# rasd3/TODA

Measured on AMD Instinct MI355X. Metric: LiDAR training samples/sec, higher is better.
Workload: dtype f32

## Files before the change

### include/toda.h

```cpp
#ifndef TODA_H_
#define TODA_H_

#include <stddef.h>
#include <stdint.h>

#ifdef __cplusplus
extern "C" {
#endif

#define TODA_OK 0
#define TODA_EINVAL (-1)
#define TODA_EWORKSPACE (-2)
#define TODA_ELAUNCH (-3)
#define TODA_EFAULT (-4)

#define TODA_FAULT_BN2D 1u
#define TODA_FAULT_WINO 2u
#define TODA_FAULT_FPS 4u

const char* toda_last_error(void);
int toda_abi_version(void);
int toda_device_fault(void);

size_t toda_voxelize_workspace_bytes(int n_points, int max_voxels);
// ... 232 lines not shown
                     const double* hi_xy_host, int closed, int32_t* flags, void* stream);
int toda_points_polar_cell(const float* points, int n, const int32_t* n_dev, int c, float phase,
                           const double* yaw_edges_host, int n_yaw, const double* dis_edges_host, int n_dis,
                           float dis_lo, float dis_hi, int32_t* cell, void* stream);
int toda_points_polar_select(const float* points, int n, const int32_t* n_dev, int c, double lo, double hi, int yaw_mode,
                             int dis_mode, double dis_th, const float* pitch_range_dev, int32_t* flags, void* stream);
size_t toda_points_pitch_range_workspace_bytes(void);
int toda_points_pitch_range(const float* points, int n, const int32_t* n_dev, int c, float* range_dev, void* ws,
                            size_t ws_bytes, void* stream);
int toda_points_pitch_band(const float* points, int n, const int32_t* n_dev, int c, float z_offset, float clip_lo,
                           float clip_hi, const double* edges_host, int n_bands, int32_t* band, void* stream);
size_t toda_rows_select_workspace_bytes(int n);
int toda_rows_select_append(const float* src, int n, const int32_t* n_dev, int c, const int32_t* keys,
                            int match, int invert, float* dst, int cap_rows, int32_t* cursor_dev,
                            void* ws, size_t ws_bytes, void* stream);
int toda_points_rotate_z(const float* src, int n, const int32_t* n_dev, int c, double cosv, double sinv,
                         float* dst, void* stream);
int toda_points_world_transform(const float* src, int n, const int32_t* n_dev, int c, int flip_x, int flip_y,
                                int rotate, float cosv, float sinv, int rescale, float scale, float* dst,
                                void* stream);

int toda_spconv_gather_gemm_stats_supported(int c_gather, int c_produce);
size_t toda_spconv_gather_gemm_stats_doubles(int n_out, int c_produce);
int toda_spconv_gather_gemm_stats(const float* in, int n_in, int c_gather, const float* packed_w, const int32_t* nbr,
                                  int n_out, int k_vol, int c_produce, const float* bias, float* out, double* sums,
                                  size_t sums_doubles, void* stream);
int toda_spconv_gather_gemm_stats_partials(const float* in, int n_in, int c_gather, const float* wp, const int32_t* nbr,
                                           int n_out, int k_vol, int c_produce, const float* bias , float* out,
                                           double* sums, size_t sums_doubles, int* blocks_out, void* stream);

int toda_conv3x3_supported(int batch, int cin, int cout, int H, int W);
size_t toda_conv3x3_weight_floats(int cout, int cin);
int toda_conv3x3_transform_weight(const float* w, int cout, int cin, int mode, float* u, void* stream);
size_t toda_conv3x3_workspace_bytes(void);
size_t toda_conv3x3_wgrad_workspace_bytes(int batch, int cin, int cout, int H, int W);
int toda_conv3x3_wgrad(const float* x, const float* dy, int batch, int cin, int cout, int H, int W, float* dw,
                       void* ws, size_t ws_bytes, void* stream);
int toda_conv3x3_fwd(const float* x, const float* u, const float* bias, int batch, int cin, int cout, int H,
                     int W, float* y, void* ws, size_t ws_bytes, void* stream);

int toda_conv3x3s2_supported(int batch, int cin, int cout, int H, int W);
int toda_conv3x3s2_fwd(const float* x, const float* w, int batch, int cin, int cout, int H, int W, float* y, void* stream);
int toda_conv3x3s2_dgrad(const float* dy, const float* w, int batch, int cin, int cout, int H, int W, float* dx, void* stream);
size_t toda_conv3x3s2_wgrad_workspace_bytes(int batch, int cin, int cout, int H, int W);
int toda_conv3x3s2_wgrad(const float* x, const float* dy, int batch, int cin, int cout, int H, int W, float* dw, void* ws,
                         size_t ws_bytes, void* stream);
int toda_deconv_supported(int batch, int cin, int cout, int H, int W, int s);
int toda_deconv_fwd(const float* x, const float* w, int batch, int cin, int cout, int H, int W, int s, float* y, void* stream);
int toda_deconv_dgrad(const float* dy, const float* w, int batch, int cin, int cout, int H, int W, int s, float* dx, void* stream);
size_t toda_deconv_wgrad_workspace_bytes(int batch, int cin, int cout, int H, int W, int s);
int toda_deconv_wgrad(const float* x, const float* dy, int batch, int cin, int cout, int H, int W, int s, float* dw, void* ws,
                      size_t ws_bytes, void* stream);

size_t toda_center_loss_workspace_bytes(int batch, int classes, int H, int W, int max_objs, int code_size);
int toda_center_loss_fwd(const float* hm_logits, const float* heatmap, int batch, int classes, int H, int W, int n_branch,
                         const float* const* reg_maps_host, const int32_t* reg_channels_host, const int64_t* inds,
                         const int64_t* mask, const float* target_boxes, int max_objs, int code_size,
                         const float* code_weights_host, float cls_weight, float loc_weight, float* hm_prob, float* out4,
                         void* ws, size_t ws_bytes, void* stream);
int toda_center_loss_bwd(const float* out4, const float* up_hm, const float* up_loc, int batch, int classes, int H, int W,
                         int n_branch, float* const* reg_grads_host, const int32_t* reg_channels_host, const int64_t* inds,
                         const int64_t* mask, int max_objs, int code_size, const float* code_weights_host, float cls_weight, float loc_weight,
                         float* hm_grad, const void* ws, size_t ws_bytes, void* stream);

int toda_conv3x3_narrow_supported(int batch, int cin, int cout, int H, int W);
int toda_conv3x3_narrow_fwd(int n, const float* const* x_host, const float* const* w_host, const float* const* bias_host,
// ... 37 lines not shown
```

### toda_amd/csrc/conv2d.hip

```cpp
#include <hip/hip_ext.h>
#include <stdlib.h>

#include "common.h"

#ifndef TODA_ABLATE
#define TODA_ABLATE 0
#endif

namespace toda {

typedef float f32x4 __attribute__((ext_vector_type(4)));
typedef float f32x2 __attribute__((ext_vector_type(2)));
typedef unsigned int u32x4w __attribute__((ext_vector_type(4)));

constexpr int WN_BLOCK = 256;
constexpr int WN_TILES = 32;
constexpr int WN_COUT = 32;
constexpr int WN_KC = 8;
constexpr int WN_FREQ = 36;
constexpr int WN_IMG = 256;
constexpr unsigned WN_OOB = 0xFFFFFFF0u;

struct WinoGeom {
    int B, Cin, Cout, H, W;
    int tiles_x, tiles_y, tiles_img, n_tiles;
    int n_tile_blocks, n_cout_blocks, n_chunks;
};

__device__ __constant__ double WN_G[6][3] = {
    {1.0, 0.0, 0.0},
    {-1.0 / 3, 1.0 / 3, -1.0 / 3},
    {1.0 / 3, 1.0 / 3, 1.0 / 3},
    {-16.0 / 15, -8.0 / 15, -4.0 / 15},
    {1.0 / 15, -2.0 / 15, 4.0 / 15},
// ... 1 lines not shown
};

__device__ __forceinline__ void wn_bt(float d0, float d1, float d2, float d3, float d4, float d5, float& v0, float& v1,
                                      float& v2, float& v3, float& v4, float& v5) {
    const float a = d3 - d1, b = d4 - d2;
    v0 = __builtin_fmaf(1.5f, a, __builtin_fmaf(-2.0f, d2, d0 + d4));
    v1 = __builtin_fmaf(-2.5f, d2, __builtin_fmaf(0.5f, d3, d1 + d4));
    v2 = __builtin_fmaf(2.5f, d3, __builtin_fmaf(0.5f, d2, d4 - d1));
    v3 = __builtin_fmaf(2.0f, a, b);
    v4 = __builtin_fmaf(-0.5f, a, b);
    v5 = __builtin_fmaf(1.5f, b, __builtin_fmaf(-2.0f, d3, d1 + d5));
}

__device__ __forceinline__ void wn_at(float m0, float m1, float m2, float m3, float m4, float m5, float& y0, float& y1,
                                      float& y2, float& y3) {
    const float s = m1 + m2, d = m2 - m1;
    y0 = (m0 + s) + (m3 + m4);
    y1 = __builtin_fmaf(-2.0f, m4, __builtin_fmaf(0.5f, m3, d));
    y2 = __builtin_fmaf(4.0f, m4, __builtin_fmaf(0.25f, m3, s));
    y3 = __builtin_fmaf(-8.0f, m4, __builtin_fmaf(0.125f, m3, d)) + m5;
}

__device__ __forceinline__ void wn_a(float y0, float y1, float y2, float y3, float& m0, float& m1, float& m2, float& m3,
                                     float& m4, float& m5) {
    const float e = y0 + y2, o = y1 + y3;
    m0 = y0;
    m1 = e - o;
    m2 = e + o;
    m3 = __builtin_fmaf(0.125f, y3, __builtin_fmaf(0.25f, y2, __builtin_fmaf(0.5f, y1, y0)));
    m4 = __builtin_fmaf(-8.0f, y3, __builtin_fmaf(4.0f, y2, __builtin_fmaf(-2.0f, y1, y0)));
    m5 = y3;
}

__global__ void __launch_bounds__(WN_BLOCK)
wino_weight_kernel(const float* __restrict__ w, int cout, int cin, int mode, float* __restrict__ u) {
    const unsigned per = (unsigned)6 * cout * cin;
    unsigned e = blockIdx.x * WN_BLOCK + threadIdx.x;
    if (e >= (mode == 2 ? 2 * per : per)) return;
    const int md = mode == 2 ? (e >= per ? 1 : 0) : mode;
    float* dst = u;
    if (e >= per) {
        e -= per;
        dst += (size_t)WN_FREQ * cout * cin;
    }
    const int CI = md ? cout : cin;
    const unsigned n_chunks = (unsigned)CI >> 3;
    const int s_ = (int)(e & 1), n = (int)((e >> 1) & 15), j = (int)((e >> 5) & 3), wc = (int)((e >> 7) & 1);
    unsigned t = e >> 8;
    const int fi = (int)(t % 6u);
    t /= 6u;
    const int chunk = (int)(t % n_chunks), cb = (int)(t / n_chunks);
    const int co = cb * 32 + wc * 16 + n, ci = chunk * 8 + 2 * j + s_;
    const float* const gp = w + (md ? ((size_t)ci * cin + co) : ((size_t)co * cin + ci)) * 9;
    double tb[3];
#pragma unroll
    for (int b2 = 0; b2 < 3; ++b2) {
        double acc = 0.0;
#pragma unroll
        for (int a = 0; a < 3; ++a) acc += WN_G[fi][a] * (double)(md ? gp[(2 - a) * 3 + (2 - b2)] : gp[a * 3 + b2]);
        tb[b2] = acc;
    }
    dst += ((size_t)(cb * n_chunks + chunk) * WN_FREQ + fi * 6) * WN_IMG + (e & 255u);
#pragma unroll
    for (int fj = 0; fj < 6; ++fj) dst[(size_t)fj * WN_IMG] = (float)(tb[0] * WN_G[fj][0] + tb[1] * WN_G[fj][1] + tb[2] * WN_G[fj][2]);
}

__device__ __forceinline__ __amdgpu_buffer_rsrc_t wn_rsrc(const float* base, unsigned bytes) {
    return __builtin_amdgcn_make_buffer_rsrc(const_cast<float*>(base), 0, bytes, 0x00020000);
}

__device__ __forceinline__ int wn_work_id() {
    const int nwg = gridDim.x, xcd = blockIdx.x & 7, q8 = nwg >> 3, r8 = nwg & 7;
    return (xcd < r8 ? xcd * (q8 + 1) : r8 * (q8 + 1) + (xcd - r8) * q8) + (blockIdx.x >> 3);
}

struct PatchOff {
    unsigned offc[6];
    unsigned offe[6];
    bool left, right;
    bool tail;
};

__device__ __forceinline__ PatchOff wn_patch_off(int tile, int t, int chan, int C, const WinoGeom& g) {
    PatchOff p;
    const bool exists = tile < g.n_tiles;
    const int tl = exists ? tile : 0;
    const int b = tl / g.tiles_img, rem = tl - b * g.tiles_img;
    const int ty = rem / g.tiles_x, tx = rem - ty * g.tiles_x;
    const int y0 = 4 * ty, x0 = 4 * tx;
    const int base = ((b * C + chan) * g.H + (y0 - 1)) * g.W + x0;
    const bool has_l = x0 > 0, has_r = x0 + 4 < g.W;
    p.left = has_l || t == 0;
    p.right = has_r || t == 15;
    p.tail = x0 + 3 >= g.W;
#pragma unroll
    for (int r = 0; r < 6; ++r) {
        const int yy = y0 - 1 + r;
// ... 701 lines not shown
                float* const d0 = lds + buf * IMG + img_off;
                float* const d1 = lds + (2 + buf) * IMG + img_off;
#pragma unroll
                for (int f = 0; f < WN_FREQ; ++f) {
                    d0[f * WN_IMG] = st.x.c[f % 6][f & 3];
                    d1[f * WN_IMG] = st.y.c[f & 3][f % 4];
                }
                return;
            }
            wn_x_transform_store(st.x, lds + buf * IMG + img_off);
            wn_dy_transform_store(st.y, lds + (2 + buf) * IMG + img_off);
        };
        auto barrier = [&]() { asm volatile("s_waitcnt lgkmcnt(0)\n\ts_barrier" ::: "memory"); };
        WStage s0, s1;
        fetch(s0, 0);
        fetch(s1, 1);
        produce(s0, 0);
        int q = 0;
        while (true) {
            barrier();
            if (q + 1 >= total) break;
            fetch(s0, q + 2);
            produce(s1, (q + 1) & 1);
            ++q;
            barrier();
            if (q + 1 >= total) break;
            fetch(s1, q + 2);
            produce(s0, (q + 1) & 1);
            ++q;
        }
    }
}

template <int SLAB>
__global__ void __launch_bounds__(WN_BLOCK)
wino_wgrad_reduce_kernel(const float* __restrict__ slabs, const int n_units, const int steps_per_unit, int G, float* __restrict__ red) {
    static_assert(SLAB % WN_BLOCK == 0, "a fold block must not straddle two units");
    __shared__ int seg[WS_MAX_GRID];
    __shared__ int n_seg;
    const long long e = (long long)blockIdx.x * WN_BLOCK + threadIdx.x;
    const int unit = (int)(((long long)blockIdx.x * WN_BLOCK) / SLAB);
    if (threadIdx.x == 0) {
        const long long S = (long long)n_units * steps_per_unit;
        const long long u_lo = (long long)unit * steps_per_unit, u_hi = u_lo + steps_per_unit;
        int w0 = (int)(u_lo * G / S);
        while (w0 > 0 && ws_range_lo(w0, G, S) > u_lo) --w0;
        while (w0 + 1 < G && ws_range_lo(w0 + 1, G, S) <= u_lo) ++w0;
        int n = 0;
        long long lo = ws_range_lo(w0, G, S);
        for (int w = w0; w < G && lo < u_hi; ++w) {
            const long long next = ws_range_lo(w + 1, G, S);
            if (next > u_lo && next != lo) seg[n++] = w;
            lo = next;
        }
        n_seg = n;
    }
    __syncthreads();
    if (unit >= n_units) return;
    const int off = (int)(e - (long long)unit * SLAB);
    const float* p = slabs + (size_t)unit * SLAB + off;
    const int n = n_seg;
    float acc = 0.0f;
    int i = 0;
    for (; i + 8 <= n; i += 8) {
        float v[8];
#pragma unroll
        for (int j = 0; j < 8; ++j) v[j] = p[(size_t)seg[i + j] * SLAB];
#pragma unroll
        for (int j = 0; j < 8; ++j) acc += v[j];
    }
    for (; i < n; ++i) acc += p[(size_t)seg[i] * SLAB];
    red[e] = acc;
}

__global__ void __launch_bounds__(WN_BLOCK)
wino_wgrad_finish_kernel(const float* __restrict__ red, const WgradGeom wg, float* __restrict__ dw) {
    const int e = blockIdx.x * WN_BLOCK + threadIdx.x;
    const int cin = wg.g.Cin, cout = wg.g.Cout;
    if (e >= cin * cout) return;
    const int co = e / cin, ci = e - co * cin;
    const int unit = (ci >> 5) * wg.n_co_blocks + (co >> 5);
    const float* sl = red + (size_t)unit * WG_SLAB_FLOATS + (co & 31) * 32 + (ci & 31);
    double du[WN_FREQ];
#pragma unroll
    for (int f = 0; f < WN_FREQ; ++f) du[f] = (double)sl[f * 1024];
    double t[3][6];
#pragma unroll
    for (int a = 0; a < 3; ++a)
#pragma unroll
        for (int j = 0; j < 6; ++j) {
            double acc = 0.0;
#pragma unroll
            for (int i = 0; i < 6; ++i) acc += WN_G[i][a] * du[i * 6 + j];
            t[a][j] = acc;
        }
    float* out = dw + ((size_t)co * cin + ci) * 9;
#pragma unroll
    for (int a = 0; a < 3; ++a)
#pragma unroll
        for (int b = 0; b < 3; ++b) {
            double acc = 0.0;
#pragma unroll
            for (int j = 0; j < 6; ++j) acc += t[a][j] * WN_G[j][b];
            out[a * 3 + b] = (float)acc;
        }
}


static int wino_geom(const char* who, int batch, int cin, int cout, int H, int W, WinoGeom* g) {
    TODA_CHECK_ARG(batch >= 1 && H >= 1 && W >= 2 && W % 2 == 0, "%s: needs batch >= 1, H >= 1 and an even W (got %d x %d x %d)", who, batch, H, W);
    TODA_CHECK_ARG(cin >= WN_KC && cin % WN_KC == 0, "%s: input channels must be a multiple of %d (got %d)", who, WN_KC, cin);
    TODA_CHECK_ARG(cout >= WN_COUT && cout % WN_COUT == 0, "%s: output channels must be a multiple of %d (got %d)", who, WN_COUT, cout);
    const long long in_bytes = 4LL * batch * cin * H * W, out_bytes = 4LL * batch * cout * H * W;
    TODA_CHECK_ARG(in_bytes < (1LL << 32) - 65536 && out_bytes < (1LL << 32) - 65536, "%s: tensor above 4 GiB", who);
    g->B = batch, g->Cin = cin, g->Cout = cout, g->H = H, g->W = W;
    g->tiles_x = (W + 3) / 4, g->tiles_y = (H + 3) / 4;
    g->tiles_img = g->tiles_x * g->tiles_y;
    g->n_tiles = batch * g->tiles_img;
    g->n_tile_blocks = cdiv(g->n_tiles, WN_TILES);
    g->n_cout_blocks = cout / WN_COUT;
    g->n_chunks = cin / WN_KC;
    return TODA_OK;
}

}

using namespace toda;

extern "C" size_t toda_conv3x3_weight_floats(int cout, int cin) {
    return (size_t)WN_FREQ * cout * cin;
}

extern "C" int toda_conv3x3_supported(int batch, int cin, int cout, int H, int W) {
    if (batch < 1 || H < 1 || W < 2 || (W & 1)) return 0;
    if (cin < 32 || cin % 32 || cout < 32 || cout % 32) return 0;
    if (4LL * batch * (cin > cout ? cin : cout) * H * W >= (1LL << 32) - 65536) return 0;
    return 1;
}

extern "C" int toda_conv3x3_transform_weight(const float* w, int cout, int cin, int mode, float* u, void* stream) {
    TODA_CHECK_ARG(w && u && mode >= 0 && mode <= 2, "conv3x3_transform_weight: null pointer or bad mode");
    const int CO = mode == 1 ? cin : cout, CI = mode == 1 ? cout : cin;
    TODA_CHECK_ARG(CO % WN_COUT == 0 && CI % WN_KC == 0 && CO > 0 && CI > 0 && (mode != 2 || (CI % WN_COUT == 0)),
                   "conv3x3_transform_weight: produced channels %% 32 and contracted channels %% 8 must be 0 (got %d, %d)", CO, CI);
    const long long threads = 6LL * cout * cin * (mode == 2 ? 2 : 1);
    TODA_CHECK_ARG(threads * 6 < (1LL << 31), "conv3x3_transform_weight: operand above 2^31 elements");
    hipLaunchKernelGGL(wino_weight_kernel, dim3(cdiv(threads, WN_BLOCK)), dim3(WN_BLOCK), 0, (hipStream_t)stream, w, cout, cin, mode, u);
    TODA_LAUNCH_CHECK();
    return TODA_OK;
}

extern "C" size_t toda_conv3x3_workspace_bytes(void) {
    return WS_FLAG_BYTES + (size_t)WS_MAX_GRID * WS_SLAB_FLOATS * sizeof(float);
}

extern "C" int toda_conv3x3_fwd(const float* x, const float* u, const float* bias, int batch, int cin, int cout, int H, int W,
                                float* y, void* ws, size_t ws_bytes, void* stream) {
    TODA_CHECK_ARG(x && u && y, "conv3x3_fwd: null pointer");
    WinoGeom g;
    int rc = wino_geom("conv3x3_fwd", batch, cin, cout, H, W, &g);
    if (rc) return rc;
    static const int variant = getenv("TODA_WINO_VARIANT") ? atoi(getenv("TODA_WINO_VARIANT")) : 1;
    const int n_units = g.n_tile_blocks * g.n_cout_blocks;
    if (variant == 0) {
        hipLaunchKernelGGL(wino_fwd_kernel, dim3(n_units), dim3(WN_BLOCK), 0, (hipStream_t)stream, x, u, bias, y, g);
    } else {
        TODA_CHECK_ARG(ws != nullptr, "conv3x3_fwd: workspace missing");
        if (ws_bytes < toda_conv3x3_workspace_bytes()) {
            toda::set_error("conv3x3_fwd: workspace too small (%zu < %zu bytes)", ws_bytes, toda_conv3x3_workspace_bytes());
            return TODA_EWORKSPACE;
        }
        static int n_cu = 0;
        if (!n_cu) {
            int dev = 0;
            hipDeviceProp_t prop;
            TODA_HIP(hipGetDevice(&dev));
            TODA_HIP(hipGetDeviceProperties(&prop, dev));
            n_cu = prop.multiProcessorCount > 0 ? prop.multiProcessorCount : 256;
            if (n_cu > WS_MAX_GRID) n_cu = WS_MAX_GRID;
        }
        static const int env_gang = getenv("TODA_WINO_GANG") ? atoi(getenv("TODA_WINO_GANG")) : 1;
        static const int gang_kb = getenv("TODA_WINO_GANG_KB") ? atoi(getenv("TODA_WINO_GANG_KB")) : 2560;
// ... 37 lines not shown


extern "C" size_t toda_conv3x3_wgrad_workspace_bytes(int batch, int cin, int cout, int H, int W) {
    (void)batch, (void)H, (void)W;
    const size_t units = (size_t)(cin / 32) * (cout / 32);
    return (WS_MAX_GRID + 2 * units) * WG_SLAB_FLOATS * sizeof(float);
}

extern "C" int toda_conv3x3_wgrad(const float* x, const float* dy, int batch, int cin, int cout, int H, int W, float* dw, void* ws,
                                  size_t ws_bytes, void* stream) {
    TODA_CHECK_ARG(x && dy && dw, "conv3x3_wgrad: null pointer");
    WgradGeom wg;
    int rc = wgrad_geom("conv3x3_wgrad", batch, cin, cout, H, W, &wg);
    if (rc) return rc;
    const size_t need = toda_conv3x3_wgrad_workspace_bytes(batch, cin, cout, H, W);
    if (!ws || ws_bytes < need) {
        toda::set_error("conv3x3_wgrad: workspace too small (%zu < %zu bytes)", ws_bytes, need);
        return TODA_EWORKSPACE;
    }
    static int n_cu = 0;
    if (!n_cu) {
        int dev = 0;
        hipDeviceProp_t prop;
        TODA_HIP(hipGetDevice(&dev));
        TODA_HIP(hipGetDeviceProperties(&prop, dev));
        n_cu = prop.multiProcessorCount > 0 ? prop.multiProcessorCount : 256;
        if (n_cu > WS_MAX_GRID) n_cu = WS_MAX_GRID;
    }
    const long long steps = (long long)wg.n_units * wg.steps_per_unit;
    const int grid = steps < n_cu ? (int)steps : n_cu;
    static const int ablate = (TODA_ABLATE && getenv("TODA_WINO_WG_ABLATE")) ? atoi(getenv("TODA_WINO_WG_ABLATE")) : 0;
    hipLaunchKernelGGL(wino_wgrad_kernel, dim3(grid), dim3(WS_BLOCK), 0, (hipStream_t)stream, x, dy, wg, (float*)ws, ablate);
    TODA_LAUNCH_CHECK();
    float* red = (float*)ws + (size_t)(WS_MAX_GRID + wg.n_units) * WG_SLAB_FLOATS;
    hipLaunchKernelGGL(wino_wgrad_reduce_kernel<WG_SLAB_FLOATS>, dim3(cdiv((long long)wg.n_units * WG_SLAB_FLOATS, WN_BLOCK)), dim3(WN_BLOCK), 0,
                       (hipStream_t)stream, (const float*)ws, wg.n_units, wg.steps_per_unit, grid, red);
    TODA_LAUNCH_CHECK();
    hipLaunchKernelGGL(wino_wgrad_finish_kernel, dim3(cdiv((long long)cin * cout, WN_BLOCK)), dim3(WN_BLOCK), 0, (hipStream_t)stream,
                       (const float*)red, wg, dw);
    TODA_LAUNCH_CHECK();
    return TODA_OK;
}
```

### toda_amd/lib.py

```python
import ctypes as C
import os

import torch

_HERE = os.path.dirname(os.path.abspath(__file__))
LIB_PATH = os.environ.get("TODA_HIP_LIB") or os.path.join(_HERE, "libtoda_hip.so")

_vp, _i, _sz, _dbl = C.c_void_p, C.c_int, C.c_size_t, C.c_double

SIGNATURES = {
    "toda_last_error": (C.c_char_p, []),
    "toda_abi_version": (_i, []),
    "toda_device_fault": (_i, []),
    "toda_voxelize_workspace_bytes": (_sz, [_i, _i]),
    "toda_voxelize_hard": (_i, [_vp, _i, _i, _vp, _vp, _vp, _i, _i, _vp, _vp, _vp, _vp, _vp, _sz, _vp]),
    "toda_mean_vfe_fwd": (_i, [_vp, _vp, _i, _i, _i, _vp, _vp]),
    "toda_mean_vfe_bwd": (_i, [_vp, _vp, _i, _i, _i, _vp, _vp]),
    "toda_dynvox_workspace_bytes": (_sz, [_i, _i, _vp, _i]),
    "toda_dynvox_count": (_i, [_vp, _i, _i, _i, _vp, _vp, _vp, _i, _vp, _vp, _sz, _vp]),
    "toda_dynvox_index": (_i, [_vp, _i, _i, _i, _vp, _vp, _vp, _i, _i, _i, _vp, _vp, _vp, _vp, _vp, _vp, _vp, _vp, _sz, _vp]),
    "toda_dynvox_seg_sum": (_i, [_vp, _i, _i, _i, _vp, _vp, _vp, _i, _i, _vp, _vp]),
    "toda_dynvox_pillar_decorate": (_i, [_vp, _i, _vp, _vp, _vp, _vp, _i, _vp, _vp, _i, _i, _vp, _i, _vp]),
    "toda_dynvox_seg_max_fwd": (_i, [_vp, _i, _vp, _vp, _i, _vp, _vp, _vp]),
    "toda_dynvox_seg_max_bwd": (_i, [_vp, _vp, _i, _i, _i, _vp, _vp]),
# ... 71 lines not shown
    "toda_voxel_pool_table": (_i, [_vp, _vp, _i, _i, _i, _vp, _vp, _vp, _sz, _vp]),
    "toda_voxel_pool_bwd_feat": (_i, [_vp, _vp, _i, _i, _i, _vp, _vp, _i, _vp, _vp]),
    "toda_voxel_pool_bwd_pos_doubles": (_sz, [_i]),
    "toda_voxel_pool_bwd_pos": (_i, [_vp, _vp, _vp, _vp, _i, _i, _i, _vp, _i, _vp, _vp, _vp, _vp]),
    "toda_fps_resident_blocks": (_i, []),
    "toda_fps_workspace_bytes": (_sz, [_i, _i]),
    "toda_fps": (_i, [_vp, _vp, _i, _i, _i, _vp, _vp, _vp, _sz, _vp]),
    "toda_ball_query_stack": (_i, [_vp, _i, _vp, _vp, _vp, _i, _i, _i, _vp, _vp, _vp, _vp, _vp]),
    "toda_sa_gather_fwd": (_i, [_vp, _i, _i, _vp, _vp, _vp, _i, _i, _vp, _vp, _vp, _vp]),
    "toda_sa_gather_bwd_feat": (_i, [_vp, _i, _i, _i, _vp, _vp, _i, _vp, _vp]),
    "toda_sa_gather_bwd_pos_doubles": (_sz, [_i]),
    "toda_sa_gather_bwd_pos": (_i, [_vp, _vp, _vp, _i, _i, _i, _vp, _i, _vp, _vp, _vp, _vp]),
    "toda_sa_max_fwd": (_i, [_vp, _i, _i, _i, _vp, _vp, _vp]),
    "toda_sa_max_bwd": (_i, [_vp, _vp, _i, _i, _i, _vp, _vp]),
    "toda_bev_interp_fwd": (_i, [_vp, _i, _i, _i, _i, _vp, _vp, _i, _vp, _vp, _vp, _vp]),
    "toda_bev_interp_bwd": (_i, [_vp, _i, _i, _vp, _vp, _vp, _i, _i, _i, _vp, _vp]),
    "toda_clip_adam_chunk": (_i, []),
    "toda_clip_adam_step": (_i, [_vp, _vp, _vp, _vp, _vp, _vp, _vp, _i, _vp, _vp, C.c_float, C.c_float, C.c_float, C.c_float, C.c_float, C.c_float, _i, _vp]),
    "toda_points_in_boxes": (_i, [_vp, _i, _vp, _i, _vp, _i, _i, _i, _vp, _vp]),
    "toda_points_sector": (_i, [_vp, _i, _vp, _i, _dbl, _dbl, _vp, _vp]),
    "toda_points_rect": (_i, [_vp, _i, _vp, _i, _vp, _vp, _i, _vp, _vp]),
    "toda_points_polar_cell": (_i, [_vp, _i, _vp, _i, C.c_float, _vp, _i, _vp, _i, C.c_float, C.c_float, _vp, _vp]),
    "toda_points_polar_select": (_i, [_vp, _i, _vp, _i, _dbl, _dbl, _i, _i, _dbl, _vp, _vp, _vp]),
    "toda_points_pitch_range_workspace_bytes": (_sz, []),
    "toda_points_pitch_range": (_i, [_vp, _i, _vp, _i, _vp, _vp, _sz, _vp]),
    "toda_points_pitch_band": (_i, [_vp, _i, _vp, _i, C.c_float, C.c_float, C.c_float, _vp, _i, _vp, _vp]),
    "toda_rows_select_workspace_bytes": (_sz, [_i]),
    "toda_rows_select_append": (_i, [_vp, _i, _vp, _i, _vp, _i, _i, _vp, _i, _vp, _vp, _sz, _vp]),
    "toda_points_rotate_z": (_i, [_vp, _i, _vp, _i, _dbl, _dbl, _vp, _vp]),
    "toda_points_world_transform": (_i, [_vp, _i, _vp, _i, _i, _i, _i, C.c_float, C.c_float, _i, C.c_float, _vp, _vp]),
    "toda_conv3x3_supported": (_i, [_i, _i, _i, _i, _i]),
    "toda_conv3x3_weight_floats": (_sz, [_i, _i]),
    "toda_conv3x3_transform_weight": (_i, [_vp, _i, _i, _i, _vp, _vp]),
    "toda_conv3x3_workspace_bytes": (_sz, []),
    "toda_conv3x3_wgrad_workspace_bytes": (_sz, [_i, _i, _i, _i, _i]),
    "toda_conv3x3_wgrad": (_i, [_vp, _vp, _i, _i, _i, _i, _i, _vp, _vp, _sz, _vp]),
    "toda_conv3x3_fwd": (_i, [_vp, _vp, _vp, _i, _i, _i, _i, _i, _vp, _vp, _sz, _vp]),
    "toda_conv3x3_narrow_supported": (_i, [_i, _i, _i, _i, _i]),
    "toda_conv3x3_narrow_fwd": (_i, [_i, _vp, _vp, _vp, _vp, _i, _i, _i, _i, C.c_longlong, _vp, _vp]),
    "toda_conv3x3_narrow_dgrad": (_i, [_i, _vp, _vp, _vp, _i, _i, _i, _i, C.c_longlong, _vp, _vp]),
    "toda_conv3x3_narrow_wgrad_workspace_bytes": (_sz, [_i, _i, _i, _i]),
    "toda_conv3x3_narrow_wgrad": (_i, [_i, _vp, _vp, _vp, _i, _i, _i, _i, C.c_longlong, _vp, _vp, _sz, _vp]),
    "toda_center_loss_workspace_bytes": (_sz, [_i, _i, _i, _i, _i, _i]),
    "toda_center_loss_fwd": (_i, [_vp, _vp, _i, _i, _i, _i, _i, _vp, _vp, _vp, _vp, _vp, _i, _i, _vp, C.c_float, C.c_float, _vp, _vp, _vp, _sz, _vp]),
    "toda_center_loss_bwd": (_i, [_vp, _vp, _vp, _i, _i, _i, _i, _i, _vp, _vp, _vp, _vp, _i, _i, _vp, C.c_float, C.c_float, _vp, _vp, _sz, _vp]),
    "toda_timing_begin": (_i, [_i]),
    "toda_timing_end": (_i, [_vp, _i, _vp]),
    "toda_center_assign": (_i, [_vp, _i, _i, _i, _i, _i, _i, _vp, _vp, _i, _i, _dbl, _i, _vp, _vp, _vp, _vp, _vp]),
    "toda_anchor_assign_workspace_bytes": (_sz, [_i, _i]),
    "toda_anchor_assign": (_i, [_vp, _vp, _vp, _vp, _vp, _i, _i, _vp, _i, _i, _i, _vp, _i, _i, _i, _i, _vp, _vp, _vp, _vp, _sz, _vp]),
    "toda_eval_overlaps": (_i, [_vp, _vp, _vp, _vp, _vp, _vp, _vp, _i, C.c_longlong, _i, _i, _vp, _vp]),
    "toda_eval_match_workspace_bytes": (_sz, [_i, _i, _i]),
    "toda_eval_match_scores": (_i, [_vp, _vp, _vp, _vp, _vp, _vp, _vp, _i, _i, _dbl, _vp, _vp, _vp, _sz, _vp]),
    "toda_eval_match": (_i, [_vp, _vp, _vp, _vp, _vp, _vp, _vp, _vp, _vp, _vp, _vp, _vp, _i, _i, _vp, _i, _dbl, _i, _i, _vp, _vp, _sz, _vp]),
}

_lib = None


def load():
    global _lib
    if _lib is not None:
        return _lib
    if not os.path.exists(LIB_PATH):
        raise RuntimeError(
            f"{LIB_PATH} not found: build it with `python -c 'import __graft_entry__ as g; g.build()'` "
# ... 38 lines not shown


def stream():
    if _raw_stream is not None and _raw_device is not None:
        return _raw_stream(_raw_device())
    return torch.cuda.current_stream().cuda_stream


def host_ptrs(tensors):
    return (C.c_void_p * len(tensors))(*[ptr(t) for t in tensors])


def host_addrs(addrs):
    return (C.c_void_p * len(addrs))(*[int(a) for a in addrs])


def host_i32(vals):
    arr = (C.c_int32 * len(vals))(*[int(v) for v in vals])
    return arr


def host_f32(vals):
    arr = (C.c_float * len(vals))(*[float(v) for v in vals])
    return arr


def host_f64(vals):
    arr = (C.c_double * len(vals))(*[float(v) for v in vals])
    return arr


def hptr(arr):
    return C.cast(arr, C.c_void_p)
```

### toda_amd/ops.py

```python
import numpy as np
import torch

from . import arena as _arena
from . import lib as L


def _triple(v):
    if isinstance(v, (list, tuple)):
        assert len(v) == 3
        return [int(x) for x in v]
    return [int(v)] * 3


def grid_size_xyz(pc_range, voxel_size):
    r = np.asarray(pc_range, dtype=np.float64)
    return np.round((r[3:6] - r[0:3]) / np.asarray(voxel_size, dtype=np.float64)).astype(np.int64)


import os as _os
import time as _time

_COUNT_PINNED = {}
_LAST_WAIT_S = 0.0

# ... 1090 lines not shown
BN2D_CAT = _os.environ.get("TODA_BN2D_CAT", "1") == "1"


def bn2d_supported(x, bn):
    if not (FUSED_BN2D and type(bn) is torch.nn.BatchNorm2d and bn.training and bn.affine and bn.track_running_stats and bn.momentum is not None):
        return False
    if not (x.is_cuda and x.dtype == torch.float32 and x.dim() == 4 and x.is_contiguous()):
        return False
    return bool(L.load().toda_bn2d_supported(x.shape[0], x.shape[1], x.shape[2] * x.shape[3]))


def bn2d(x, bn, relu):
    bump_bn_counter(bn)
    return _BN2d.apply(x, bn.weight, bn.bias, bn.running_mean, bn.running_var, bn.momentum, bn.eps, relu)


def bn2d_cat(pairs, relu=True):
    flat = []
    for x, bn in pairs:
        bump_bn_counter(bn)
        flat += [x, bn.weight, bn.bias, bn.running_mean, bn.running_var, bn.momentum, bn.eps]
    return _BN2dCat.apply(relu, len(pairs), *flat)


def bn_relu_tail(seq):
    mods = list(seq)
    if len(mods) >= 2 and type(mods[-1]) is torch.nn.ReLU and type(mods[-2]) is torch.nn.BatchNorm2d:
        return mods[:-2], mods[-2]
    return None


def run_dense_sequential(seq, x):
    mods = list(seq)
    i = 0
    while i < len(mods):
        m = mods[i]
        if isinstance(m, torch.nn.Sequential):
            x = run_dense_sequential(m, x)
        elif (type(m) is torch.nn.ZeroPad2d and tuple(m.padding) == (1, 1, 1, 1) and i + 1 < len(mods) and type(mods[i + 1]) is torch.nn.Conv2d
              and mods[i + 1].padding == (0, 0) and conv3x3_supported(x, mods[i + 1])):
            x = conv3x3(x, mods[i + 1].weight, mods[i + 1].bias)
            i += 2
            continue
        elif (type(m) is torch.nn.ZeroPad2d and tuple(m.padding) == (1, 1, 1, 1) and i + 1 < len(mods) and conv3x3s2_supported(x, mods[i + 1])):
            x = conv3x3s2(x, mods[i + 1].weight, mods[i + 1].bias)
            i += 2
            continue
        elif deconv_supported(x, m):
            x = deconv(x, m.weight, m.stride[0], m.bias)
        elif type(m) is torch.nn.Conv2d and m.padding == (1, 1) and conv3x3_supported(x, m):
            x = conv3x3(x, m.weight, m.bias)
        elif type(m) is torch.nn.BatchNorm2d and bn2d_supported(x, m):
            relu = i + 1 < len(mods) and type(mods[i + 1]) is torch.nn.ReLU
            x = bn2d(x, m, relu)
            i += 2 if relu else 1
            continue
        elif type(m) is torch.nn.BatchNorm2d and x.is_cuda and m.track_running_stats and m.momentum is not None:
            bump_bn_counter(m)
            x = torch.nn.functional.batch_norm(x, m.running_mean, m.running_var, m.weight, m.bias, m.training, m.momentum, m.eps)
        else:
            x = m(x)
        i += 1
    return x


DENSE_CONV = _os.environ.get("TODA_DENSE_CONV", "winograd")
_WINO_CACHE = {}


def conv3x3_supported(x, conv):
    if DENSE_CONV != "winograd" or type(conv) is not torch.nn.Conv2d or not x.is_cuda or x.dtype != torch.float32 or x.dim() != 4:
        return False
    if conv.kernel_size != (3, 3) or conv.stride != (1, 1) or conv.dilation != (1, 1) or conv.groups != 1:
        return False
    if conv.padding_mode != "zeros" or conv.in_channels != x.shape[1]:
        return False
    b, c, h, w = x.shape
    return bool(L.load().toda_conv3x3_supported(b, conv.in_channels, conv.out_channels, h, w))


def conv3x3_transform_weight(weight, mode):
    lib = L.load()
    cout, cin = weight.shape[0], weight.shape[1]
    n = lib.toda_conv3x3_weight_floats(cout, cin)
    u = torch.empty((2, n) if mode == 2 else (n,), dtype=torch.float32, device=weight.device)
    L.check(lib.toda_conv3x3_transform_weight(L.ptr(weight.contiguous()), cout, cin, int(mode), L.ptr(u), L.stream()),
            "toda_conv3x3_transform_weight")
    return u


def _conv3x3_workspace(device):
    key = (device.index, L.stream())
    ws = _WINO_CACHE.get(key)
    if ws is None:
        ws = _WINO_CACHE[key] = torch.zeros((L.load().toda_conv3x3_workspace_bytes(),), dtype=torch.uint8, device=device)
    return ws


def conv3x3_run(x, u, bias, cout):
    lib = L.load()
    b, cin, h, w = x.shape
    y = torch.empty((b, cout, h, w), dtype=torch.float32, device=x.device)
    ws = _conv3x3_workspace(x.device)
    L.check(lib.toda_conv3x3_fwd(L.ptr(x), L.ptr(u), L.ptr(bias), b, cin, cout, h, w, L.ptr(y), L.ptr(ws), ws.numel(), L.stream()),
            "toda_conv3x3_fwd")
    return y


class _Conv3x3(torch.autograd.Function):

    @staticmethod
    def forward(ctx, x, weight, bias):
        x = x.contiguous()
        need_dx = ctx.needs_input_grad[0]
        u = conv3x3_transform_weight(weight, 2 if need_dx else 0)
        y = conv3x3_run(x, u[0] if need_dx else u, bias, weight.shape[0])
        ctx.save_for_backward(x, weight, u[1] if need_dx else None)
        ctx.has_bias = bias is not None
        return y

    @staticmethod
    def backward(ctx, gy):
        x, weight, u_dgrad = ctx.saved_tensors
        gy = gy.contiguous()
        gx = gw = gb = None
        if ctx.needs_input_grad[0]:
            gx = conv3x3_run(gy, u_dgrad if u_dgrad is not None else conv3x3_transform_weight(weight, 1), None, weight.shape[1])
        if ctx.needs_input_grad[1]:
            gw = conv3x3_wgrad(x, gy, weight.shape)
        if ctx.has_bias and ctx.needs_input_grad[2]:
            gb = gy.sum((0, 2, 3))
        return gx, gw, gb


def conv3x3_wgrad(x, gy, wshape):
    lib = L.load()
    b, cin, h, w = x.shape
    cout = gy.shape[1]
    dw = torch.empty(tuple(wshape), dtype=torch.float32, device=x.device)
    ws_bytes = lib.toda_conv3x3_wgrad_workspace_bytes(b, cin, cout, h, w)
    ws = torch.empty((max(ws_bytes, 16),), dtype=torch.uint8, device=x.device)
    L.check(lib.toda_conv3x3_wgrad(L.ptr(x), L.ptr(gy), b, cin, cout, h, w, L.ptr(dw), L.ptr(ws), ws_bytes, L.stream()),
            "toda_conv3x3_wgrad")
    return dw


def conv3x3(x, weight, bias=None):
    return _Conv3x3.apply(x, weight, bias)


class _Conv3x3S2(torch.autograd.Function):

    @staticmethod
    def forward(ctx, x, weight):
        lib = L.load()
        x, weight = x.contiguous(), weight.contiguous()
        b, cin, h, w = x.shape
        cout = weight.shape[0]
        y = torch.empty((b, cout, h // 2, w // 2), dtype=torch.float32, device=x.device)
        L.check(lib.toda_conv3x3s2_fwd(L.ptr(x), L.ptr(weight), b, cin, cout, h, w, L.ptr(y), L.stream()), "toda_conv3x3s2_fwd")
        ctx.save_for_backward(x, weight)
        return y

    @staticmethod
    def backward(ctx, gy):
        x, weight = ctx.saved_tensors
        lib = L.load()
        gy = gy.contiguous()
        b, cin, h, w = x.shape
        cout = weight.shape[0]
        gx = gw = None
        if ctx.needs_input_grad[0]:
            gx = torch.empty_like(x)
            L.check(lib.toda_conv3x3s2_dgrad(L.ptr(gy), L.ptr(weight), b, cin, cout, h, w, L.ptr(gx), L.stream()), "toda_conv3x3s2_dgrad")
        if ctx.needs_input_grad[1]:
            gw = torch.empty_like(weight)
            nb = lib.toda_conv3x3s2_wgrad_workspace_bytes(b, cin, cout, h, w)
            ws = torch.empty((max(nb, 16),), dtype=torch.uint8, device=x.device)
            L.check(lib.toda_conv3x3s2_wgrad(L.ptr(x), L.ptr(gy), b, cin, cout, h, w, L.ptr(gw), L.ptr(ws), nb, L.stream()), "toda_conv3x3s2_wgrad")
        return gx, gw

# ... 862 lines not shown
```

### toda_amd/pcdet/models/backbones_2d/base_bev_backbone.py

```python
import numpy as np
import torch
import torch.nn as nn

from toda_amd import ops


def _bn(c):
    return nn.BatchNorm2d(c, eps=1e-3, momentum=0.01)


class BaseBEVBackbone(nn.Module):
    def __init__(self, model_cfg, input_channels):
        super().__init__()
        self.model_cfg = model_cfg
        layer_nums = list(model_cfg.get("LAYER_NUMS", None) or [])
        layer_strides = list(model_cfg.get("LAYER_STRIDES", None) or [])
        num_filters = list(model_cfg.get("NUM_FILTERS", None) or [])
        assert len(layer_nums) == len(layer_strides) == len(num_filters)
        up_strides = list(model_cfg.get("UPSAMPLE_STRIDES", None) or [])
        up_filters = list(model_cfg.get("NUM_UPSAMPLE_FILTERS", None) or [])
        assert len(up_strides) == len(up_filters)

        self.blocks, self.deblocks = nn.ModuleList(), nn.ModuleList()
        c_prev = input_channels
        for lvl, (n_layers, stride, width) in enumerate(zip(layer_nums, layer_strides, num_filters)):
            seq = [nn.ZeroPad2d(1), nn.Conv2d(c_prev, width, 3, stride=stride, padding=0, bias=False), _bn(width),
                   nn.ReLU()]
            for _ in range(n_layers):
                seq += [nn.Conv2d(width, width, 3, padding=1, bias=False), _bn(width), nn.ReLU()]
            self.blocks.append(nn.Sequential(*seq))
            c_prev = width
            if up_strides:
                s = up_strides[lvl]
                if s >= 1:
                    up = nn.ConvTranspose2d(width, up_filters[lvl], s, stride=s, bias=False)
                else:
                    k = int(np.round(1 / s))
                    up = nn.Conv2d(width, up_filters[lvl], k, stride=k, bias=False)
                self.deblocks.append(nn.Sequential(up, _bn(up_filters[lvl]), nn.ReLU()))
        c_cat = sum(up_filters)
        if len(up_strides) > len(layer_nums):
            s = up_strides[-1]
            self.deblocks.append(nn.Sequential(nn.ConvTranspose2d(c_cat, c_cat, s, stride=s, bias=False), _bn(c_cat),
                                               nn.ReLU()))
        self.num_bev_features = c_cat

    def forward(self, data_dict):
        x = data_dict["spatial_features"]
        if getattr(self, "dense_channels_last", False):
            x = x.contiguous(memory_format=torch.channels_last)
        h0 = x.shape[2]
        ups, pre = [], []
        tails = [ops.bn_relu_tail(d) for d in self.deblocks[:len(self.blocks)]] if (ops.BN2D_CAT and len(self.blocks) > 1 and len(self.deblocks) >= len(self.blocks)) else []
        for lvl, block in enumerate(self.blocks):
            x = ops.run_dense_sequential(block, x)
            data_dict[f"spatial_features_{int(h0 / x.shape[2])}x"] = x
            if tails and all(t is not None for t in tails):
                pre.append((ops.run_dense_sequential(tails[lvl][0], x), tails[lvl][1]))
            else:
                ups.append(ops.run_dense_sequential(self.deblocks[lvl], x) if len(self.deblocks) > 0 else x)
        if pre:
            if all(ops.bn2d_supported(z, bn) for z, bn in pre) and len({z.shape[2:] for z, _ in pre}) == 1:
                x = ops.bn2d_cat(pre, relu=True)
            else:
                ups = [torch.relu(ops.run_dense_sequential([bn], z)) for z, bn in pre]
        if len(ups) > 1:
            x = torch.cat(ups, dim=1)
        elif len(ups) == 1:
            x = ups[0]
        if len(self.deblocks) > len(self.blocks):
            x = ops.run_dense_sequential(self.deblocks[-1], x)
        data_dict["spatial_features_2d"] = x
        return data_dict
```

Measured before the change: 146.8.

## Batch Winograd weight transforms across layers and fuse wgrad reduce with filter fold

Adds a batched weight-transform kernel that handles up to 16 conv3x3 layers in one launch, plus a Python prepack pass that caches the transformed weights per conv, keyed on weight version, pointer and a manual epoch. It also adds a wgrad fold kernel that sums the per-workgroup slabs and applies the inverse filter transform in a single kernel, replacing the separate reduce and transform launches. The intent is to cut kernel launches and host overhead in the BEV backbone. The cache is invalidated only through the weight version and pointer and an explicit epoch bump, so in-place weight writes that skip the version counter could leave stale transformed weights.

```diff
diff --git a/include/toda.h b/include/toda.h
--- a/include/toda.h
+++ b/include/toda.h
@@ -288,6 +288,12 @@
 int toda_conv3x3_supported(int batch, int cin, int cout, int H, int W);
 size_t toda_conv3x3_weight_floats(int cout, int cin);
 int toda_conv3x3_transform_weight(const float* w, int cout, int cin, int mode, float* u, void* stream);
+typedef struct toda_conv3x3_weight_entry {
+    const float* w;
+    int32_t cout, cin, mode, reserved;
+    float* u;
+} toda_conv3x3_weight_entry;
+int toda_conv3x3_transform_weight_batch(const toda_conv3x3_weight_entry* table_host, int n, void* stream);
 size_t toda_conv3x3_workspace_bytes(void);
 size_t toda_conv3x3_wgrad_workspace_bytes(int batch, int cin, int cout, int H, int W);
 int toda_conv3x3_wgrad(const float* x, const float* dy, int batch, int cin, int cout, int H, int W, float* dw,
diff --git a/toda_amd/csrc/conv2d.hip b/toda_amd/csrc/conv2d.hip
--- a/toda_amd/csrc/conv2d.hip
+++ b/toda_amd/csrc/conv2d.hip
@@ -1,5 +1,6 @@
 #include <hip/hip_ext.h>
 #include <stdlib.h>
+#include <string.h>
 
 #include "common.h"
 
@@ -67,10 +68,8 @@
     m5 = y3;
 }
 
-__global__ void __launch_bounds__(WN_BLOCK)
-wino_weight_kernel(const float* __restrict__ w, int cout, int cin, int mode, float* __restrict__ u) {
+__device__ __forceinline__ void wn_weight_element(const float* __restrict__ w, int cout, int cin, int mode, float* __restrict__ u, unsigned e) {
     const unsigned per = (unsigned)6 * cout * cin;
-    unsigned e = blockIdx.x * WN_BLOCK + threadIdx.x;
     if (e >= (mode == 2 ? 2 * per : per)) return;
     const int md = mode == 2 ? (e >= per ? 1 : 0) : mode;
     float* dst = u;
@@ -98,6 +97,27 @@
     dst += ((size_t)(cb * n_chunks + chunk) * WN_FREQ + fi * 6) * WN_IMG + (e & 255u);
 #pragma unroll
     for (int fj = 0; fj < 6; ++fj) dst[(size_t)fj * WN_IMG] = (float)(tb[0] * WN_G[fj][0] + tb[1] * WN_G[fj][1] + tb[2] * WN_G[fj][2]);
+}
+
+__global__ void __launch_bounds__(WN_BLOCK)
+wino_weight_kernel(const float* __restrict__ w, int cout, int cin, int mode, float* __restrict__ u) {
+    wn_weight_element(w, cout, cin, mode, u, blockIdx.x * WN_BLOCK + threadIdx.x);
+}
+
+constexpr int WB_MAX_LAYERS = 16;
+struct WeightBatch {
+    const float* w[WB_MAX_LAYERS];
+    float* u[WB_MAX_LAYERS];
+    int cout[WB_MAX_LAYERS], cin[WB_MAX_LAYERS], mode[WB_MAX_LAYERS];
+    unsigned first_block[WB_MAX_LAYERS + 1];
+    int n;
+};
+
+__global__ void __launch_bounds__(WN_BLOCK)
+wino_weight_batch_kernel(const WeightBatch b) {
+    int l = 0;
+    while (l + 1 < b.n && blockIdx.x >= b.first_block[l + 1]) ++l;
+    wn_weight_element(b.w[l], b.cout[l], b.cin[l], b.mode[l], b.u[l], (blockIdx.x - b.first_block[l]) * WN_BLOCK + threadIdx.x);
 }
 
 __device__ __forceinline__ __amdgpu_buffer_rsrc_t wn_rsrc(const float* base, unsigned bytes) {
@@ -865,6 +885,97 @@
     }
 }
 
+__device__ __forceinline__ int wn_unit_segments(int unit, int n_units, int steps_per_unit, int G, int* __restrict__ seg) {
+    const long long S = (long long)n_units * steps_per_unit;
+    const long long u_lo = (long long)unit * steps_per_unit, u_hi = u_lo + steps_per_unit;
+    int w0 = (int)(u_lo * G / S);
+    while (w0 > 0 && ws_range_lo(w0, G, S) > u_lo) --w0;
+    while (w0 + 1 < G && ws_range_lo(w0 + 1, G, S) <= u_lo) ++w0;
+    int n = 0;
+    long long lo = ws_range_lo(w0, G, S);
+    for (int w = w0; w < G && lo < u_hi; ++w) {
+        const long long next = ws_range_lo(w + 1, G, S);
+        if (next > u_lo && next != lo) seg[n++] = w;
+        lo = next;
+    }
+    return n;
+}
+
+__device__ __forceinline__ void wn_filter_grad(const double (&du)[WN_FREQ], float* __restrict__ out) {
+    double t[3][6];
+#pragma unroll
+    for (int a = 0; a < 3; ++a)
+#pragma unroll
+        for (int j = 0; j < 6; ++j) {
+            double acc = 0.0;
+#pragma unroll
+            for (int i = 0; i < 6; ++i) acc += WN_G[i][a] * du[i * 6 + j];
+            t[a][j] = acc;
+        }
+#pragma unroll
+    for (int a = 0; a < 3; ++a)
+#pragma unroll
+        for (int b = 0; b < 3; ++b) {
+            double acc = 0.0;
+#pragma unroll
+            for (int j = 0; j < 6; ++j) acc += t[a][j] * WN_G[j][b];
+            out[a * 3 + b] = (float)acc;
+        }
+}
+
+constexpr int WF_PAIRS = 32;
+constexpr int WF_SUMS = (WN_FREQ * WF_PAIRS + WN_BLOCK - 1) / WN_BLOCK;
+
+__global__ void __launch_bounds__(WN_BLOCK)
+wino_wgrad_fold_kernel(const float* __restrict__ slabs, const WgradGeom wg, int G, float* __restrict__ dw) {
+    __shared__ int seg[WS_MAX_GRID];
+    __shared__ int n_seg;
+    __shared__ float du_s[WN_FREQ * WF_PAIRS];
+    const int tid = threadIdx.x;
+    const int unit = blockIdx.x >> 5, row = blockIdx.x & 31;
+    if (tid == 0) n_seg = wn_unit_segments(unit, wg.n_units, wg.steps_per_unit, G, seg);
+    __syncthreads();
+    const int n = n_seg;
+    const float* p[WF_SUMS];
+    float acc[WF_SUMS];
+#pragma unroll
+    for (int k = 0; k < WF_SUMS; ++k) {
+        const int idx = tid + k * WN_BLOCK < WN_FREQ * WF_PAIRS ? tid + k * WN_BLOCK : tid;
+        p[k] = slabs + (size_t)unit * WG_SLAB_FLOATS + (idx >> 5) * 1024 + row * 32 + (idx & 31);
+        acc[k] = 0.0f;
+    }
+    int i = 0;
+    for (; i + 8 <= n; i += 8) {
+        float v[WF_SUMS][8];
+#pragma unroll
+        for (int j = 0; j < 8; ++j) {
+            const size_t off = (size_t)seg[i + j] * WG_SLAB_FLOATS;
+#pragma unroll
+            for (int k = 0; k < WF_SUMS; ++k) v[k][j] = p[k][off];
+        }
+#pragma unroll
+        for (int k = 0; k < WF_SUMS; ++k)
+#pragma unroll
+            for (int j = 0; j < 8; ++j) acc[k] += v[k][j];
+    }
+    for (; i < n; ++i) {
+        const size_t off = (size_t)seg[i] * WG_SLAB_FLOATS;
+#pragma unroll
+        for (int k = 0; k < WF_SUMS; ++k) acc[k] += p[k][off];
+    }
+#pragma unroll
+    for (int k = 0; k < WF_SUMS; ++k)
+        if (tid + k * WN_BLOCK < WN_FREQ * WF_PAIRS) du_s[tid + k * WN_BLOCK] = acc[k];
+    __syncthreads();
+    if (tid >= WF_PAIRS) return;
+    double du[WN_FREQ];
+#pragma unroll
+    for (int f = 0; f < WN_FREQ; ++f) du[f] = (double)du_s[f * WF_PAIRS + tid];
+    const int cib = unit / wg.n_co_blocks, cob = unit - cib * wg.n_co_blocks;
+    const int co = cob * 32 + row, ci = cib * 32 + tid;
+    wn_filter_grad(du, dw + ((size_t)co * wg.g.Cin + ci) * 9);
+}
+
 template <int SLAB>
 __global__ void __launch_bounds__(WN_BLOCK)
 wino_wgrad_reduce_kernel(const float* __restrict__ slabs, const int n_units, const int steps_per_unit, int G, float* __restrict__ red) {
@@ -873,21 +984,7 @@
     __shared__ int n_seg;
     const long long e = (long long)blockIdx.x * WN_BLOCK + threadIdx.x;
     const int unit = (int)(((long long)blockIdx.x * WN_BLOCK) / SLAB);
-    if (threadIdx.x == 0) {
-        const long long S = (long long)n_units * steps_per_unit;
-        const long long u_lo = (long long)unit * steps_per_unit, u_hi = u_lo + steps_per_unit;
-        int w0 = (int)(u_lo * G / S);
-        while (w0 > 0 && ws_range_lo(w0, G, S) > u_lo) --w0;
-        while (w0 + 1 < G && ws_range_lo(w0 + 1, G, S) <= u_lo) ++w0;
-        int n = 0;
-        long long lo = ws_range_lo(w0, G, S);
-        for (int w = w0; w < G && lo < u_hi; ++w) {
-            const long long next = ws_range_lo(w + 1, G, S);
-            if (next > u_lo && next != lo) seg[n++] = w;
-            lo = next;
-        }
-        n_seg = n;
-    }
+    if (threadIdx.x == 0) n_seg = wn_unit_segments(unit, n_units, steps_per_unit, G, seg);
     __syncthreads();
     if (unit >= n_units) return;
     const int off = (int)(e - (long long)unit * SLAB);
@@ -917,26 +1014,7 @@
     double du[WN_FREQ];
 #pragma unroll
     for (int f = 0; f < WN_FREQ; ++f) du[f] = (double)sl[f * 1024];
-    double t[3][6];
-#pragma unroll
-    for (int a = 0; a < 3; ++a)
-#pragma unroll
-        for (int j = 0; j < 6; ++j) {
-            double acc = 0.0;
-#pragma unroll
-            for (int i = 0; i < 6; ++i) acc += WN_G[i][a] * du[i * 6 + j];
-            t[a][j] = acc;
-        }
-    float* out = dw + ((size_t)co * cin + ci) * 9;
-#pragma unroll
-    for (int a = 0; a < 3; ++a)
-#pragma unroll
-        for (int b = 0; b < 3; ++b) {
-            double acc = 0.0;
-#pragma unroll
-            for (int j = 0; j < 6; ++j) acc += t[a][j] * WN_G[j][b];
-            out[a * 3 + b] = (float)acc;
-        }
+    wn_filter_grad(du, dw + ((size_t)co * cin + ci) * 9);
 }
 
 
@@ -981,6 +1059,39 @@
     hipLaunchKernelGGL(wino_weight_kernel, dim3(cdiv(threads, WN_BLOCK)), dim3(WN_BLOCK), 0, (hipStream_t)stream, w, cout, cin, mode, u);
     TODA_LAUNCH_CHECK();
     return TODA_OK;
+}
+
+extern "C" int toda_conv3x3_transform_weight_batch(const toda_conv3x3_weight_entry* table, int n, void* stream) {
+    TODA_CHECK_ARG(n >= 0 && (table || n == 0), "conv3x3_transform_weight_batch: null table");
+    WeightBatch b = {};
+    auto flush = [&]() -> int {
+        if (b.n > 0) {
+            hipLaunchKernelGGL(wino_weight_batch_kernel, dim3(b.first_block[b.n]), dim3(WN_BLOCK), 0, (hipStream_t)stream, b);
+            TODA_LAUNCH_CHECK();
+        }
+        b.n = 0;
+        return TODA_OK;
+    };
+    for (int i = 0; i < n; ++i) {
+        const toda_conv3x3_weight_entry& t = table[i];
+        const int cout = t.cout, cin = t.cin, mode = t.mode;
+        TODA_CHECK_ARG(t.w && t.u && mode >= 0 && mode <= 2, "conv3x3_transform_weight_batch: entry %d: null pointer or bad mode", i);
+        const int CO = mode == 1 ? cin : cout, CI = mode == 1 ? cout : cin;
+        TODA_CHECK_ARG(CO % WN_COUT == 0 && CI % WN_KC == 0 && CO > 0 && CI > 0 && (mode != 2 || (CI % WN_COUT == 0)),
+                       "conv3x3_transform_weight_batch: entry %d: produced channels %% 32 and contracted channels %% 8 must be 0 (got %d, %d)", i, CO, CI);
+        const long long threads = 6LL * cout * cin * (mode == 2 ? 2 : 1);
+        TODA_CHECK_ARG(threads * 6 < (1LL << 31), "conv3x3_transform_weight_batch: entry %d: operand above 2^31 elements", i);
+        const long long blocks = cdiv(threads, WN_BLOCK);
+        if (b.n == WB_MAX_LAYERS || (b.n > 0 && b.first_block[b.n] + blocks >= (1LL << 31))) {
+            const int rc = flush();
+            if (rc) return rc;
+        }
+        b.w[b.n] = t.w, b.u[b.n] = t.u, b.cout[b.n] = cout, b.cin[b.n] = cin, b.mode[b.n] = mode;
+        if (b.n == 0) b.first_block[0] = 0;
+        b.first_block[b.n + 1] = b.first_block[b.n] + (unsigned)blocks;
+        ++b.n;
+    }
+    return flush();
 }
 
 extern "C" size_t toda_conv3x3_workspace_bytes(void) {
@@ -1084,6 +1195,13 @@
     static const int ablate = (TODA_ABLATE && getenv("TODA_WINO_WG_ABLATE")) ? atoi(getenv("TODA_WINO_WG_ABLATE")) : 0;
     hipLaunchKernelGGL(wino_wgrad_kernel, dim3(grid), dim3(WS_BLOCK), 0, (hipStream_t)stream, x, dy, wg, (float*)ws, ablate);
     TODA_LAUNCH_CHECK();
+    const char* const fold = getenv("TODA_WGRAD_FOLD");
+    if (!(fold && !strcmp(fold, "pair"))) {
+        hipLaunchKernelGGL(wino_wgrad_fold_kernel, dim3(wg.n_units * (1024 / WF_PAIRS)), dim3(WN_BLOCK), 0, (hipStream_t)stream,
+                           (const float*)ws, wg, grid, dw);
+        TODA_LAUNCH_CHECK();
+        return TODA_OK;
+    }
     float* red = (float*)ws + (size_t)(WS_MAX_GRID + wg.n_units) * WG_SLAB_FLOATS;
     hipLaunchKernelGGL(wino_wgrad_reduce_kernel<WG_SLAB_FLOATS>, dim3(cdiv((long long)wg.n_units * WG_SLAB_FLOATS, WN_BLOCK)), dim3(WN_BLOCK), 0,
                        (hipStream_t)stream, (const float*)ws, wg.n_units, wg.steps_per_unit, grid, red);
diff --git a/toda_amd/lib.py b/toda_amd/lib.py
--- a/toda_amd/lib.py
+++ b/toda_amd/lib.py
@@ -127,6 +127,7 @@
     "toda_conv3x3_supported": (_i, [_i, _i, _i, _i, _i]),
     "toda_conv3x3_weight_floats": (_sz, [_i, _i]),
     "toda_conv3x3_transform_weight": (_i, [_vp, _i, _i, _i, _vp, _vp]),
+    "toda_conv3x3_transform_weight_batch": (_i, [_vp, _i, _vp]),
     "toda_conv3x3_workspace_bytes": (_sz, []),
     "toda_conv3x3_wgrad_workspace_bytes": (_sz, [_i, _i, _i, _i, _i]),
     "toda_conv3x3_wgrad": (_i, [_vp, _vp, _i, _i, _i, _i, _i, _vp, _vp, _sz, _vp]),
@@ -231,3 +232,7 @@
 
 def hptr(arr):
     return C.cast(arr, C.c_void_p)
+
+
+class Conv3x3WeightEntry(C.Structure):
+    _fields_ = [("w", C.c_void_p), ("cout", C.c_int32), ("cin", C.c_int32), ("mode", C.c_int32), ("reserved", C.c_int32), ("u", C.c_void_p)]
diff --git a/toda_amd/ops.py b/toda_amd/ops.py
--- a/toda_amd/ops.py
+++ b/toda_amd/ops.py
@@ -1146,6 +1146,7 @@
 
 def run_dense_sequential(seq, x):
     mods = list(seq)
+    conv3x3_prepack(mods, x)
     i = 0
     while i < len(mods):
         m = mods[i]
@@ -1153,7 +1154,7 @@
             x = run_dense_sequential(m, x)
         elif (type(m) is torch.nn.ZeroPad2d and tuple(m.padding) == (1, 1, 1, 1) and i + 1 < len(mods) and type(mods[i + 1]) is torch.nn.Conv2d
               and mods[i + 1].padding == (0, 0) and conv3x3_supported(x, mods[i + 1])):
-            x = conv3x3(x, mods[i + 1].weight, mods[i + 1].bias)
+            x = conv3x3(x, mods[i + 1].weight, mods[i + 1].bias, conv3x3_prepacked(mods[i + 1]))
             i += 2
             continue
         elif (type(m) is torch.nn.ZeroPad2d and tuple(m.padding) == (1, 1, 1, 1) and i + 1 < len(mods) and conv3x3s2_supported(x, mods[i + 1])):
@@ -1163,7 +1164,7 @@
         elif deconv_supported(x, m):
             x = deconv(x, m.weight, m.stride[0], m.bias)
         elif type(m) is torch.nn.Conv2d and m.padding == (1, 1) and conv3x3_supported(x, m):
-            x = conv3x3(x, m.weight, m.bias)
+            x = conv3x3(x, m.weight, m.bias, conv3x3_prepacked(m))
         elif type(m) is torch.nn.BatchNorm2d and bn2d_supported(x, m):
             relu = i + 1 < len(mods) and type(mods[i + 1]) is torch.nn.ReLU
             x = bn2d(x, m, relu)
@@ -1203,6 +1204,79 @@
     return u
 
 
+def conv3x3_transform_weights_batched(items):
+    lib = L.load()
+    if not items:
+        return []
+    sizes = [lib.toda_conv3x3_weight_floats(w.shape[0], w.shape[1]) * (2 if mode == 2 else 1) for w, mode in items]
+    flat = torch.empty((sum(sizes),), dtype=torch.float32, device=items[0][0].device)
+    ws = [w.contiguous() for w, _ in items]
+    table = (L.Conv3x3WeightEntry * len(items))()
+    outs, off = [], 0
+    for ent, w, (_, mode), n in zip(table, ws, items, sizes):
+        u = flat[off:off + n]
+        ent.w, ent.cout, ent.cin, ent.mode, ent.u = L.ptr(w), w.shape[0], w.shape[1], int(mode), L.ptr(u)
+        outs.append(u.view(2, n // 2) if mode == 2 else u)
+        off += n
+    L.check(lib.toda_conv3x3_transform_weight_batch(L.hptr(table), len(items), L.stream()), "toda_conv3x3_transform_weight_batch")
+    return outs
+
+
+_WEIGHT_EPOCH = [0]
+
+
+def weights_written_in_place():
+    _WEIGHT_EPOCH[0] += 1
+
+
+def _conv3x3_weight_tag(weight):
+    return weight._version, weight.data_ptr(), _WEIGHT_EPOCH[0]
+
+
+def _conv3x3_stack(mods, dx, out):
+    prev = None
+    for m in mods:
+        if isinstance(m, torch.nn.Sequential):
+            dx = _conv3x3_stack(list(m), dx, out)
+        else:
+            if (type(m) is torch.nn.Conv2d and m.kernel_size == (3, 3) and m.stride == (1, 1) and m.dilation == (1, 1) and m.groups == 1
+                    and m.padding_mode == "zeros" and m.in_channels % 32 == 0 and m.out_channels % 32 == 0 and m.in_channels > 0
+                    and (m.padding == (1, 1) or (m.padding == (0, 0) and type(prev) is torch.nn.ZeroPad2d and tuple(prev.padding) == (1, 1, 1, 1)))
+                    and m.weight.is_cuda and m.weight.dtype == torch.float32):
+                out.append((m, dx))
+            if not dx and torch.is_grad_enabled() and isinstance(m, torch.nn.Module) and any(p.requires_grad for p in m.parameters(recurse=False)):
+                dx = True
+        prev = m
+    return dx
+
+
+def conv3x3_prepack(mods, x):
+    if DENSE_CONV != "winograd" or not x.is_cuda:
+        return 0
+    stack = []
+    _conv3x3_stack(mods, torch.is_grad_enabled() and x.requires_grad, stack)
+    stale = []
+    for conv, dx in stack:
+        ent = conv.__dict__.get("_wino_u")
+        tag = _conv3x3_weight_tag(conv.weight)
+        if ent is None or ent[0] != tag or (dx and ent[2] is None):
+            stale.append((conv, tag, dx))
+    if len(stale) < 2:
+        return 0
+    with torch.no_grad():
+        us = conv3x3_transform_weights_batched([(conv.weight.detach(), 2 if dx else 0) for conv, _, dx in stale])
+    for (conv, tag, dx), u in zip(stale, us):
+        conv.__dict__["_wino_u"] = (tag, u[0], u[1]) if dx else (tag, u, None)
+    return len(stale)
+
+
+def conv3x3_prepacked(conv):
+    ent = conv.__dict__.get("_wino_u")
+    if ent is not None and ent[0] == _conv3x3_weight_tag(conv.weight):
+        return ent[1], ent[2]
+    return None
+
+
 def _conv3x3_workspace(device):
     key = (device.index, L.stream())
     ws = _WINO_CACHE.get(key)
@@ -1224,12 +1298,16 @@
 class _Conv3x3(torch.autograd.Function):
 
     @staticmethod
-    def forward(ctx, x, weight, bias):
+    def forward(ctx, x, weight, bias, pre=None):
         x = x.contiguous()
         need_dx = ctx.needs_input_grad[0]
-        u = conv3x3_transform_weight(weight, 2 if need_dx else 0)
-        y = conv3x3_run(x, u[0] if need_dx else u, bias, weight.shape[0])
-        ctx.save_for_backward(x, weight, u[1] if need_dx else None)
+        if pre is not None:
+            u_fwd, u_dgrad = pre
+        else:
+            u = conv3x3_transform_weight(weight, 2 if need_dx else 0)
+            u_fwd, u_dgrad = (u[0], u[1]) if need_dx else (u, None)
+        y = conv3x3_run(x, u_fwd, bias, weight.shape[0])
+        ctx.save_for_backward(x, weight, u_dgrad if need_dx else None)
         ctx.has_bias = bias is not None
         return y
 
@@ -1244,7 +1322,7 @@
             gw = conv3x3_wgrad(x, gy, weight.shape)
         if ctx.has_bias and ctx.needs_input_grad[2]:
             gb = gy.sum((0, 2, 3))
-        return gx, gw, gb
+        return gx, gw, gb, None
 
 
 def conv3x3_wgrad(x, gy, wshape):
@@ -1259,8 +1337,8 @@
     return dw
 
 
-def conv3x3(x, weight, bias=None):
-    return _Conv3x3.apply(x, weight, bias)
+def conv3x3(x, weight, bias=None, pre=None):
+    return _Conv3x3.apply(x, weight, bias, pre)
 
 
 class _Conv3x3S2(torch.autograd.Function):
diff --git a/toda_amd/pcdet/models/backbones_2d/base_bev_backbone.py b/toda_amd/pcdet/models/backbones_2d/base_bev_backbone.py
--- a/toda_amd/pcdet/models/backbones_2d/base_bev_backbone.py
+++ b/toda_amd/pcdet/models/backbones_2d/base_bev_backbone.py
@@ -52,6 +52,7 @@
         h0 = x.shape[2]
         ups, pre = [], []
         tails = [ops.bn_relu_tail(d) for d in self.deblocks[:len(self.blocks)]] if (ops.BN2D_CAT and len(self.blocks) > 1 and len(self.deblocks) >= len(self.blocks)) else []
+        ops.conv3x3_prepack(list(self.blocks), x)
         for lvl, block in enumerate(self.blocks):
             x = ops.run_dense_sequential(block, x)
             data_dict[f"spatial_features_{int(h0 / x.shape[2])}x"] = x
```

Result: faster. 148.6, median of 6 (+1.2%).
